# tensor4all/tensor4all-rs

Measured on AMD Instinct MI355X. Metric: TCI2 full-sweep GF/s (d=30, chi=256 fp64), higher is better.
Workload: dtype f64

## Files before the change

tensor4all-rs_amd/build.py:

```python
#!/usr/bin/env python3
import os
import subprocess
import sys
from concurrent.futures import ThreadPoolExecutor

HERE = os.path.dirname(os.path.abspath(__file__))
CSRC = os.path.join(HERE, "csrc")
OUT = os.path.join(HERE, "lib")
OBJ = os.path.join(HERE, "build")
SOURCES = ["kernels_rrlu.hip", "kernels_rrlu_reg.hip", "rrlu_xcd_plan.hip", "kernels_rrlu_xcd2.hip", "kernels_rrlu_xcd2_group.hip", "kernels_rrlu_xcd2m.hip", "kernels_rrlu_wg.hip", "kernels_rrlu_wg_group.hip", "kernels_rrlu_w1.hip", "kernels_rrlu_global.hip", "kernels_pi.hip", "kernels_chain.hip", "kernels_small.hip", "kernels_dense.hip", "kernels_linalg.hip",
           "kernels_tt.hip", "kernels_mpo.hip", "pool.hip", "engine.hip", "rook.hip", "tt.hip", "mpo.hip", "globalsearch.hip", "tci2.hip", "tci2_chain.hip", "tci2_small.hip", "conversion.hip", "patching.hip", "tree.hip", "quantics.hip", "tensorops.hip", "aci.hip", "quanticstransform.hip", "capi.hip"]
FLAGS = ["--offload-arch=gfx950", "-O3", "-std=c++17", "-fPIC", "-ffp-contract=off", "-Wall", "-Wno-unused-function",
         "-fvisibility=hidden"] + os.environ.get("T4A_EXTRA_FLAGS", "").split()
FILE_FLAGS = {"kernels_dense.hip": ["-mllvm", "-amdgpu-mfma-vgpr-form=1"], "kernels_linalg.hip": ["-ffp-contract=fast"]}
HEADERS = ["common.hpp", "stdrng.hpp", "pishard.hpp", "kernels.hpp", "kernels_rrlu_xcd_common.hpp", "kernels_rrlu_w1_body.hpp", "engine.hpp", "tci2.hpp", "tt.hpp", "mpo.hpp", "globalsearch.hpp", "rook.hpp", "patching.hpp", "tree.hpp", "quantics.hpp", "tensorops.hpp", "aci.hpp", "quanticstransform.hpp", "../../include/t4a_gpu.h",
           "../../include/t4a_testfunctions.h"]


_INC_CACHE = {}


def _includes(path):
    path = os.path.normpath(path)
    if path in _INC_CACHE:
        return _INC_CACHE[path]
    _INC_CACHE[path] = set()
    found = set()
    try:
        with open(path) as f:
            text = f.read()
    except OSError:
        return found
    import re
    for inc in re.findall(r'^\s*#\s*include\s+"([^"]+)"', text, flags=re.M):
        cand = os.path.normpath(os.path.join(os.path.dirname(path), inc))
        if os.path.exists(cand):
            found.add(cand)
            found |= _includes(cand)
    _INC_CACHE[path] = found
    return found


def _newer(target, deps):
    if not os.path.exists(target):
        return True
    t = os.path.getmtime(target)
    return any(os.path.getmtime(d) > t for d in deps)


def build(force=False, verbose=True):
    hipcc = os.environ.get("HIPCC", "/opt/rocm/bin/hipcc")
    os.makedirs(OUT, exist_ok=True)
    os.makedirs(OBJ, exist_ok=True)
    stamp = os.path.join(OBJ, "flags.stamp")
    flags_now = " ".join(FLAGS) + " | " + repr(sorted(FILE_FLAGS.items()))
    try:
        with open(stamp) as f:
            flags_then = f.read()
    except OSError:
        flags_then = None
    if flags_then != flags_now:
        force = True
    hdrs = [os.path.join(CSRC, h) for h in HEADERS]
# ... 33 lines not shown
```

tensor4all-rs_amd/csrc/kernels.hpp:

```cpp
#pragma once

#include <hip/hip_runtime.h>

#include <cstddef>
#include <cstdint>

#include "../../include/t4a_testfunctions.h"

namespace t4a {

struct RrluWorkspace;

struct RrluPlan {
    int W = 1;
    int T = 256;
    int cpw = 0;
    int Mld = 0;
    size_t lds_bytes = 0;
};

RrluPlan rrlu_make_plan(int M, int N, int num_cus);

struct RrluArgs {
    const double* A;
// ... 209 lines not shown
    const int* ldim;
    const int* woff;
    int forward, use_extras;
    int one_site;
    uint64_t* ind_code;
    uint64_t* ind_acc;
    int* ind_cnt;
    int ind_cap;
    uint64_t* dep_code;
    uint64_t* dep_acc;
    int dep_cap;
    int* rowmap;
    int* dims;
    int* hdims;
    uint64_t* snap_dst;
    int* snap_cnt_dst;
    size_t snap_words;
    int n_sites;
    uint64_t* zero_a;
    size_t zero_a_words;
    uint64_t* zero_b;
    size_t zero_b_words;
};
struct ChainPrepArgs {
    int b;
    int do_build;
    int with_rowmap;
    int prev_b;
    const int* prev_iresult;
    const int* prev_rowperm;
    const int* prev_colperm;
    unsigned prev_token;
    unsigned long long* dbg;
    int defer_host_writes;
};
struct ChainWalkArgs {
    char* blocks;
    size_t block_bytes, off_piv, off_rp, off_cp, off_ts;
    double* pi;
    int n_bonds;
    int max_steps;
    double rel_tol, abs_tol;
    double* factors;
    size_t factors_stride;
    unsigned token_base;
    int timed;
    int lean_prep;
    unsigned long long* phase_ticks;
};
void chain_walk_launch(const ChainCommon& c, const FnDevice& fn, const ChainWalkArgs& w, int columns, hipStream_t stream);
void chain_indep_launch(const ChainCommon& c, int n_bonds, hipStream_t stream);
void chain_last_core_launch(const ChainCommon& c, const FnDevice& fn, double* core, int max_entries, hipStream_t stream);
void chain_prep_launch(const ChainCommon& c, const ChainPrepArgs& a, hipStream_t stream);
void chain_pi_launch(const ChainCommon& c, const FnDevice& fn, int b, int n_dep_ub, int n_ind_ub, double* out, hipStream_t stream);

constexpr int CHAIN_GROUP_MAX = 8;
struct ChainGroupSlot {
    ChainCommon c;
    FnDevice fn;
    double* pi;
};
struct ChainPrepGroupArgs {
    ChainPrepArgs a[CHAIN_GROUP_MAX];
};
void chain_indep_group_launch(const ChainGroupSlot* d_slots, int n_handles, int n_bonds, hipStream_t stream);
void chain_prep_group_launch(const ChainGroupSlot* d_slots, const ChainPrepGroupArgs& a, int n_handles, hipStream_t stream);
void chain_pi_group_launch(const ChainGroupSlot* d_slots, int n_handles, int b, int n_dep_ub, int n_ind_ub, hipStream_t stream);

struct GemmDesc {
    int m, n, k;
    const double* A; int lda; long long strideA; int transA;
    const double* B; int ldb; long long strideB; int transB;
    double* C; int ldc; long long strideC;
    double alpha, beta;
    int batch;
    int ksplit = 1;
    double* partial = nullptr;
};
void gemm_launch(const GemmDesc& d, hipStream_t stream);

constexpr int LUCI_LEFT_CORES_MAX_JOBS = 80;
constexpr int LUCI_LEFT_CORES_MAX_RANK = 16;
struct LeftCoreJob {
    const double* lu;
    const int* dims;
    const int* iresult;
    const int* row_perm;
    double* core;
    int S;
    unsigned token;
};
struct LeftCoreJobs {
    LeftCoreJob j[LUCI_LEFT_CORES_MAX_JOBS];
};
void luci_left_cores_batched_launch(const LeftCoreJobs& jobs, int n_jobs, int max_rows, hipStream_t stream);
bool luci_factors_small_launch(const double* lu, int M, int N, int rk, const int* row_perm, const int* col_perm, bool left_orth,
                               double* left, double* right, hipStream_t stream);
void transpose_launch(const double* in, int rows, int cols, int ldi, double* out, int ldo, hipStream_t stream);

struct TrsmProblem {
    const double* T; int ldt; int n;
    double* B; int ldb; int nrhs;
    int lower; int unit_diag;
    const int* skip_flag;
};
void trsm_left_batched_launch(const TrsmProblem* d_problems, int n_problems, int max_n, int max_nrhs, hipStream_t stream);

struct LuProblem {
    double* A; int lda; int n;
    int* piv;
    int* info;
    double* B; int ldb; int nrhs;
    const unsigned long long* pmax_bits;
};
void lu_batched_launch(const LuProblem* d_problems, int n_problems, int max_n, hipStream_t stream);
constexpr int LU_MAX_PANEL_STEPS = 128;
bool lu_forward_blocked_launch(const LuProblem* d_problems, int n_problems, int max_n, int max_nrhs, hipStream_t stream, int avoid_xcc = -1,
                               unsigned* tickets = nullptr);
bool lu_solve_blocked_launch(const LuProblem* d_problems, int n_problems, int max_n, int max_nrhs, hipStream_t stream, int avoid_xcc = -1,
                             unsigned* tickets = nullptr);
// ... 118 lines not shown
```

tensor4all-rs_amd/csrc/kernels_chain.hip:

```cpp
#include "kernels.hpp"
#include "kernels_rrlu_w1_body.hpp"

namespace t4a {

namespace {

__device__ __forceinline__ const char* chain_kernarg_base()
{
#if defined(__HIP_DEVICE_COMPILE__)
    return (const char*)__builtin_amdgcn_kernarg_segment_ptr();
#else
    return nullptr;
#endif
}

constexpr int CHAIN_T = 1024;
constexpr int WALK_T = 1024;
constexpr int CHAIN_HASH = 4096;

__device__ __forceinline__ unsigned chain_hash(unsigned long long c)
{
    c ^= c >> 33;
    c *= 0xff51afd7ed558ccdull;
    c ^= c >> 29;
// ... 300 lines not shown

__device__ __forceinline__ void chain_pi_body(const ChainCommon& c, const FnDevice& fn, int b, double* __restrict__ out)
{
    const int* dm = c.dims + (size_t)b * 4;
    if (dm[2] != 0) return;
    const int K = fn.n_acc;
    const int nd = c.forward ? dm[0] : dm[1], ni = c.forward ? dm[1] : dm[0];
    const int i = blockIdx.x * blockDim.x + threadIdx.x;
    if (blockIdx.x * (int)blockDim.x >= nd) return;
    uint64_t racc[T4A_FN_MAX_ACC] = {0, 0, 0, 0};
    if (i < nd)
        for (int k = 0; k < K; ++k) racc[k] = c.dep_acc[(size_t)i * K + k];
    const uint64_t* ia = c.ind_acc + (size_t)b * c.ind_cap * K;
    for (int j = blockIdx.y; j < ni; j += gridDim.y) {
        if (i < nd) {
            uint64_t acc[T4A_FN_MAX_ACC] = {0, 0, 0, 0};
            for (int k = 0; k < K; ++k) acc[k] = racc[k] + ia[(size_t)j * K + k];
            out[(size_t)j * nd + i] = t4a_fn_value(fn.fid, acc, fn.params);
        }
    }
}
__global__ void __launch_bounds__(256) chain_pi_kernel(ChainCommon c, FnDevice fn, int b, double* __restrict__ out) { chain_pi_body(c, fn, b, out); }
__global__ void __launch_bounds__(256) chain_pi_group_kernel(const ChainGroupSlot* __restrict__ slots, int b)
{
    const ChainGroupSlot& s = slots[blockIdx.z];
    chain_pi_body(s.c, s.fn, b, s.pi);
}


__device__ __forceinline__ void chain_mirror_body(const ChainCommon& c, int nb)
{
    const int K = c.K;
    const size_t cap = (size_t)c.cap;
    const int gtid = (int)(blockIdx.x * blockDim.x + threadIdx.x), gsz = (int)(gridDim.x * blockDim.x);
    const int lane = (int)(threadIdx.x & 63), gwave = gtid >> 6, nwaves = gsz >> 6;
    for (int pf = gwave; pf < 2 * (nb + 1); pf += nwaves) {
        const int site = pf >> 1, fam = pf & 1;
        if ((fam == 0 && site == 0) || (fam == 1 && site == nb)) continue;
        const ChainTab& T = fam == 0 ? c.I : c.J;
        const ChainTab& Mr = fam == 0 ? c.mI : c.mJ;
        const int cnt = __hip_atomic_load(T.cnt + site, __ATOMIC_RELAXED, __HIP_MEMORY_SCOPE_AGENT);
        if (cnt < 0 || cnt > c.cap) continue;
        for (int e = lane; e < cnt * (1 + K); e += 64) {
            if (e < cnt) Mr.code[(size_t)site * cap + e] = T.code[(size_t)site * cap + e];
            else Mr.acc[(size_t)site * cap * K + (e - cnt)] = T.acc[(size_t)site * cap * K + (e - cnt)];
        }
        if (lane == 0) Mr.cnt[site] = cnt;
    }
    if (c.hdims)
        for (int e = gtid; e < nb * 4; e += gsz)
            if ((e & 3) != 3) c.hdims[e] = __hip_atomic_load(c.dims + e, __ATOMIC_RELAXED, __HIP_MEMORY_SCOPE_AGENT);
}

__global__ void __launch_bounds__(256) chain_last_core_kernel(ChainCommon c, FnDevice fn, double* __restrict__ core, int max_entries)
{
    const int site = c.n_sites - 1, K = c.K;
    const size_t cap = (size_t)c.cap;
    const int L = c.I.cnt[site], R = c.J.cnt[site], S = c.ldim[site], woff = c.woff[site];
    if (L < 1 || L > c.cap || R < 1 || R > c.cap || S < 1) return;
    const long long total = (long long)L * S * R;
    if (total > (long long)max_entries) return;
    for (long long e = (long long)blockIdx.x * blockDim.x + threadIdx.x; e < total; e += (long long)gridDim.x * blockDim.x) {
        const int l = (int)(e % L), s_ = (int)((e / L) % S), r = (int)(e / ((long long)L * S));
        uint64_t acc[T4A_FN_MAX_ACC] = {0, 0, 0, 0};
        for (int q = 0; q < K; ++q)
            acc[q] = c.I.acc[((size_t)site * cap + l) * K + q] + c.w[(size_t)q * c.total + woff + s_] + c.J.acc[((size_t)site * cap + r) * K + q];
        core[e] = t4a_fn_value(fn.fid, acc, fn.params);
    }
}

__device__ __forceinline__ void walk_phase_barrier(bool scalar_cache = true)
{
    if (scalar_cache) {
        __syncthreads();
        __builtin_amdgcn_s_dcache_inv();
        asm volatile("s_waitcnt lgkmcnt(0)" ::: "memory");
    } else {
        asm volatile("s_waitcnt lgkmcnt(0)\n\ts_barrier" ::: "memory");
    }
}
__device__ __forceinline__ int walk_div_small(int x, float rd) { return (int)(((float)x + 0.5f) * rd); }
__device__ __forceinline__ int walk_load_i32(const int* p) { return __hip_atomic_load(p, __ATOMIC_RELAXED, __HIP_MEMORY_SCOPE_AGENT); }

template <bool FORWARD>
__device__ __forceinline__ void walk_prep_wave0(const ChainCommon& c, WalkShared* ws, int b, int prev_b, unsigned prev_token, bool do_build, unsigned long long* dbg = nullptr)
{
    const unsigned long long dbg_t0 = dbg ? wall_clock64() : 0ull;
    const int lane = threadIdx.x & 63;
    const int K = c.K;
    const size_t cap = (size_t)c.cap;
    bool poison = false;
    int np = 0;
    if (prev_b >= 0) {
        const int pb = prev_b;
        const int pm = ws->dims[pb * 4], pn = ws->dims[pb * 4 + 1];
        const bool bad = ws->dims[pb * 4 + 2] != 0 || ws->prev_ires[1] != 0 || ws->prev_ires[3] != (int)prev_token || pm <= 0 || pn <= 0;
        const int r = ws->prev_ires[0];
        const int cnt = r > 0 ? r : 1;
        if (bad || cnt > c.cap || cnt > pm || cnt > pn || cnt > WALK_MAX_LIST) {
            poison = true;
        } else {
            const uint64_t* const pind_code = ws->ind_code[pb & 1];
            const uint64_t* const pind_acc = ws->ind_acc[pb & 1];
            uint64_t rc = 0, cc = 0, ra[T4A_FN_MAX_ACC] = {0, 0, 0, 0}, ca[T4A_FN_MAX_ACC] = {0, 0, 0, 0};
            if (lane < cnt) {
                const int ri = r > 0 ? ws->perm_rp[lane] : 0, ci = r > 0 ? ws->perm_cp[lane] : 0;
// ... 261 lines not shown
            if (tid == 0) {
                ws->prev_ires[0] = npiv >= 0 ? npiv : 0;
                ws->prev_ires[1] = npiv >= 0 ? 0 : 1;
                ws->prev_ires[2] = 0;
                ws->prev_ires[3] = npiv >= 0 ? (int)(w.token_base + (unsigned)k) : 0;
            }
        }
        walk_phase_barrier(!w.lean_prep);
        phase(2);
    }
    for (int e = tid; e < nb * 4; e += (int)blockDim.x) c.dims[e] = ws->dims[e];
    __threadfence();
    __syncthreads();
    chain_mirror_body(c, nb);
    if (w.phase_ticks && tid == 0) {
        for (int i = 0; i < 3; ++i) w.phase_ticks[i] = ph[i];
        w.phase_ticks[3] = wall_clock64() - ph_t0;
    }
}

template <int NC, bool FORWARD, bool FACTORS> void chain_walk_launch_one(const ChainCommon& c, const FnDevice& fn, const ChainWalkArgs& w, hipStream_t stream)
{
    constexpr size_t lds = walk_lds_bytes<NC, FACTORS>();
    static std::once_flag attr_once;
    std::call_once(attr_once, [] {
        (void)hipFuncSetAttribute(reinterpret_cast<const void*>(&chain_walk_kernel<NC, FORWARD, FACTORS>), hipFuncAttributeMaxDynamicSharedMemorySize, (int)lds);
    });
    hipLaunchKernelGGL((chain_walk_kernel<NC, FORWARD, FACTORS>), dim3(1), dim3(WALK_T), lds, stream, c, fn, w);
}

template <int NC> void chain_walk_launch_nc(const ChainCommon& c, const FnDevice& fn, const ChainWalkArgs& w, hipStream_t stream)
{
    if (w.factors) {
        if (c.forward) chain_walk_launch_one<NC, true, true>(c, fn, w, stream);
        else chain_walk_launch_one<NC, false, true>(c, fn, w, stream);
    } else {
        if (c.forward) chain_walk_launch_one<NC, true, false>(c, fn, w, stream);
        else chain_walk_launch_one<NC, false, false>(c, fn, w, stream);
    }
}

}

void chain_indep_launch(const ChainCommon& c, int n_bonds, hipStream_t stream)
{
    hipLaunchKernelGGL(chain_indep_kernel, dim3(n_bonds), dim3(CHAIN_T), 0, stream, c);
}

void chain_prep_launch(const ChainCommon& c, const ChainPrepArgs& a, hipStream_t stream)
{
    hipLaunchKernelGGL(chain_prep_kernel, dim3(1), dim3(CHAIN_T), 0, stream, c, a);
}

void chain_pi_launch(const ChainCommon& c, const FnDevice& fn, int b, int n_dep_ub, int n_ind_ub, double* out, hipStream_t stream)
{
    if (n_dep_ub <= 0 || n_ind_ub <= 0) return;
    const int gy = n_ind_ub < 2048 ? n_ind_ub : 2048;
    hipLaunchKernelGGL(chain_pi_kernel, dim3((n_dep_ub + 255) / 256, gy), dim3(256), 0, stream, c, fn, b, out);
}

void chain_indep_group_launch(const ChainGroupSlot* d_slots, int n_handles, int n_bonds, hipStream_t stream)
{
    hipLaunchKernelGGL(chain_indep_group_kernel, dim3(n_bonds, n_handles), dim3(CHAIN_T), 0, stream, d_slots);
}

void chain_prep_group_launch(const ChainGroupSlot* d_slots, const ChainPrepGroupArgs& a, int n_handles, hipStream_t stream)
{
    hipLaunchKernelGGL(chain_prep_group_kernel, dim3(n_handles), dim3(CHAIN_T), 0, stream, d_slots, a);
}

void chain_pi_group_launch(const ChainGroupSlot* d_slots, int n_handles, int b, int n_dep_ub, int n_ind_ub, hipStream_t stream)
{
    if (n_dep_ub <= 0 || n_ind_ub <= 0 || n_handles <= 0) return;
    const int gy = n_ind_ub < 2048 ? n_ind_ub : 2048;
    hipLaunchKernelGGL(chain_pi_group_kernel, dim3((n_dep_ub + 255) / 256, gy, n_handles), dim3(256), 0, stream, d_slots, b);
}

void chain_walk_launch(const ChainCommon& c, const FnDevice& fn, const ChainWalkArgs& w, int columns, hipStream_t stream)
{
    if (columns <= 8) chain_walk_launch_nc<8>(c, fn, w, stream);
    else if (columns <= 16) chain_walk_launch_nc<16>(c, fn, w, stream);
    else chain_walk_launch_nc<32>(c, fn, w, stream);
}

void chain_last_core_launch(const ChainCommon& c, const FnDevice& fn, double* core, int max_entries, hipStream_t stream)
{
    const int blocks = max_entries > 256 * 64 ? 64 : (max_entries + 255) / 256;
    hipLaunchKernelGGL(chain_last_core_kernel, dim3(blocks > 0 ? blocks : 1), dim3(256), 0, stream, c, fn, core, max_entries);
}

}
```

tensor4all-rs_amd/csrc/kernels_rrlu_xcd2.hip:

```cpp
#include "kernels_rrlu_xcd_common.hpp"

namespace t4a {

namespace {

template <int RPT, int KX = 1> struct Xcd2Lds {
    static constexpr int LSTR = xcd_lstr(RPT);
    static constexpr int TBL = xcd2_tbl(RPT, KX);
    static constexpr int o_l = 0;
    static constexpr int o_wd = o_l + 64 * LSTR * 8;
    static constexpr int o_wi = o_wd + 16;
    static constexpr int o_pp = o_wi + 64;
    static constexpr int o_st = o_pp + 16;
    static constexpr int o_pv = o_st + 128;
    static constexpr int o_pr = o_pv + TBL * 8;
    static constexpr int o_rp = o_pr + TBL * 2;
    static constexpr int o_pc = o_rp + TBL * 2;
    static constexpr int o_cp = o_pc + TBL * 2;
    static constexpr int bytes = o_cp + TBL * 2;
};
static_assert(Xcd2Lds<12>::bytes == (int)xcd_lds_total(12), "plan.lds_bytes must cover the layout");
static_assert(Xcd2Lds<24>::bytes == (int)xcd2_lds_total(24), "plan.lds_bytes must cover the layout (plans beyond 1024 rows)");
static_assert(Xcd2Lds<16, 3>::bytes == (int)xcd2_lds_total(16, 3), "plan.lds_bytes must cover the layout (plans beyond 1024 columns)");

#ifndef T4A_XCD_STAMP_WAVE
#define T4A_XCD_STAMP_WAVE 0
#endif

constexpr unsigned X2_META_VALID = 1u << 13;
constexpr unsigned X2_ROW_MASK = 2047u;
constexpr int X2_QSHIFT = 11, X2_PSHIFT = 11;

constexpr int X2_DIVW = XWAVES - 1;

template <int RPT, int CPT, bool ROWMAJOR, int KX = 1>
__device__ __forceinline__ void rrlu_xcd2_body(const RrluXcdArgs& p, const RrluXcdArgs* pk)
{
    static_assert(XWAVES == 8, "the second-generation kernel is written for eight waves per workgroup");
    static_assert(KX >= 1 && KX <= 3, "instantiated for up to three XCDs");
    constexpr int ST_AUX = KX > 1 ? BUF_SC1 : 0;
    extern __shared__ __attribute__((aligned(16))) char smem_raw[];
    using L = Xcd2Lds<RPT, KX>;
    constexpr int LSTR = L::LSTR;
    constexpr int MP = 64 * RPT;
    double* const lbuf = reinterpret_cast<double*>(smem_raw + L::o_l);
    int* const ctl = reinterpret_cast<int*>(smem_raw + L::o_wi);
    unsigned long long* const lds_ptrs = reinterpret_cast<unsigned long long*>(smem_raw + L::o_pp);
    unsigned long long* const lds_stamps = reinterpret_cast<unsigned long long*>(smem_raw + L::o_st);
    double* const lds_pivots = reinterpret_cast<double*>(smem_raw + L::o_pv);
    unsigned short* const posrow = reinterpret_cast<unsigned short*>(smem_raw + L::o_pr);
    unsigned short* const rowpos = reinterpret_cast<unsigned short*>(smem_raw + L::o_rp);
    unsigned short* const poscol = reinterpret_cast<unsigned short*>(smem_raw + L::o_pc);
    unsigned short* const colpos = reinterpret_cast<unsigned short*>(smem_raw + L::o_cp);

    const int tid = threadIdx.x;
    const int lane = tid & 63;
    const int wave = __builtin_amdgcn_readfirstlane(tid >> 6);
    const unsigned long long t_entry = (kXcdStamps && p.stamps) ? __builtin_amdgcn_s_memtime() : 0ull;

    if (tid == 0) {
        int rank = -1;
        if constexpr (KX == 1) {
            if ((int)xcc_id() == p.xcc) {
                const unsigned t = atomicAdd(p.ticket, 1u) - p.ticket_base;
                if (t < (unsigned)p.W) rank = (int)t;
            }
        } else {
            const unsigned x = xcc_id() & 7u;
            const unsigned t = atomicAdd(p.ticket + x, 1u) - p.ticket_base;
            const unsigned xi = (x - (unsigned)p.xcc) & 7u;
            if (xi < (unsigned)KX && t < (unsigned)p.W) rank = (int)(xi * (unsigned)p.W + t);
        }
        ctl[3] = rank;
        ctl[0] = 0;
// ... 882 lines not shown
{
    if (a.tie_row_major) xcd2_launch_tie<RPT, CPT, true>(plan, a, stream);
    else xcd2_launch_tie<RPT, CPT, false>(plan, a, stream);
}

template <int RPT> void xcd2_launch_r(const RrluXcdPlan& plan, const RrluXcdArgs& a, hipStream_t stream)
{
    switch (plan.CPT) {
    case 1: xcd2_launch_rc<RPT, 1>(plan, a, stream); break;
    case 2: xcd2_launch_rc<RPT, 2>(plan, a, stream); break;
    case 3: if constexpr (RPT * 3 <= XCD_MAX_VALUES) xcd2_launch_rc<RPT, 3>(plan, a, stream); break;
    default: if constexpr (RPT * 4 <= XCD_MAX_VALUES) xcd2_launch_rc<RPT, 4>(plan, a, stream); break;
    }
}

#else
template <int RPT, int CPT, bool ROWMAJOR>
__global__ void __launch_bounds__(XT) __attribute__((amdgpu_waves_per_eu(XWAVES / 4, XWAVES / 4))) rrlu_xcd2_group_kernel(RrluXcdGroupArgs g)
{
    (void)g;
    const unsigned x = (unsigned)__builtin_amdgcn_readfirstlane((int)xcc_id()) & 7u;
    const RrluXcdArgs* const slot = reinterpret_cast<const RrluXcdArgs*>(kernarg_base() + (size_t)x * sizeof(RrluXcdArgs));
    rrlu_xcd2_body<RPT, CPT, ROWMAJOR>(*slot, slot);
}

template <int RPT, int CPT, bool ROWMAJOR> void xcd2_group_launch_tie(const RrluXcdPlan& plan, const RrluXcdGroupArgs& a, hipStream_t stream)
{
    static std::once_flag attr_once;
    std::call_once(attr_once, [] {
        (void)hipFuncSetAttribute(reinterpret_cast<const void*>(&rrlu_xcd2_group_kernel<RPT, CPT, ROWMAJOR>),
                                  hipFuncAttributeMaxDynamicSharedMemorySize, 160 * 1024);
    });
    hipLaunchKernelGGL((rrlu_xcd2_group_kernel<RPT, CPT, ROWMAJOR>), dim3(plan.grid), dim3(XT), plan.lds_bytes, stream, a);
}
template <int RPT, int CPT> void xcd2_group_launch_rc(const RrluXcdPlan& plan, const RrluXcdGroupArgs& a, bool row_major, hipStream_t stream)
{
    if (row_major) xcd2_group_launch_tie<RPT, CPT, true>(plan, a, stream);
    else xcd2_group_launch_tie<RPT, CPT, false>(plan, a, stream);
}
template <int RPT> void xcd2_group_launch_r(const RrluXcdPlan& plan, const RrluXcdGroupArgs& a, bool row_major, hipStream_t stream)
{
    switch (plan.CPT) {
    case 1: xcd2_group_launch_rc<RPT, 1>(plan, a, row_major, stream); break;
    case 2: xcd2_group_launch_rc<RPT, 2>(plan, a, row_major, stream); break;
    case 3: if constexpr (RPT * 3 <= XCD_MAX_VALUES) xcd2_group_launch_rc<RPT, 3>(plan, a, row_major, stream); break;
    default: if constexpr (RPT * 4 <= XCD_MAX_VALUES) xcd2_group_launch_rc<RPT, 4>(plan, a, row_major, stream); break;
    }
}

#endif

}

#if defined(T4A_XCD2_MULTI_TU)
void rrlu_xcd2m_launch(const RrluXcdPlan& plan, const RrluXcdArgs& a, hipStream_t stream)
{
    const bool ok = xcd2m_launch_rc<24, 1, 1>(plan, a, stream) || xcd2m_launch_rc<24, 2, 1>(plan, a, stream) ||
                    xcd2m_launch_rc<16, 2, 3>(plan, a, stream) || xcd2m_launch_rc<24, 2, 3>(plan, a, stream) ||
                    xcd2m_launch_rc<16, 3, 2>(plan, a, stream) || xcd2m_launch_rc<24, 2, 2>(plan, a, stream);
    if (!ok) throw std::runtime_error("no kernel instantiation for this multi-XCD rrLU plan");
}
#elif !defined(T4A_XCD_GROUP_TU)
void rrlu_xcd2_launch(const RrluXcdPlan& plan, const RrluXcdArgs& a, hipStream_t stream)
{
    switch (plan.RPT) {
#ifdef T4A_XCD_DEV
    case 2: xcd2_launch_r<2>(plan, a, stream); break;
    default: xcd2_launch_r<12>(plan, a, stream); break;
#else
    case 1: xcd2_launch_r<1>(plan, a, stream); break;
    case 2: xcd2_launch_r<2>(plan, a, stream); break;
    case 3: xcd2_launch_r<3>(plan, a, stream); break;
    case 4: xcd2_launch_r<4>(plan, a, stream); break;
    case 6: xcd2_launch_r<6>(plan, a, stream); break;
    case 8: xcd2_launch_r<8>(plan, a, stream); break;
    case 12: xcd2_launch_r<12>(plan, a, stream); break;
    default: xcd2_launch_r<16>(plan, a, stream); break;
#endif
    }
}
#else
void rrlu_xcd2_group_launch(const RrluXcdPlan& plan, const RrluXcdGroupArgs& a, bool tie_row_major, hipStream_t stream)
{
    switch (plan.RPT) {
    case 1: xcd2_group_launch_r<1>(plan, a, tie_row_major, stream); break;
    case 2: xcd2_group_launch_r<2>(plan, a, tie_row_major, stream); break;
    case 3: xcd2_group_launch_r<3>(plan, a, tie_row_major, stream); break;
    case 4: xcd2_group_launch_r<4>(plan, a, tie_row_major, stream); break;
    case 6: xcd2_group_launch_r<6>(plan, a, tie_row_major, stream); break;
    case 8: xcd2_group_launch_r<8>(plan, a, tie_row_major, stream); break;
    case 12: xcd2_group_launch_r<12>(plan, a, tie_row_major, stream); break;
    default: xcd2_group_launch_r<16>(plan, a, tie_row_major, stream); break;
    }
}
#endif

}
```

tensor4all-rs_amd/csrc/rrlu_xcd_plan.hip:

```cpp
#include "kernels_rrlu_xcd_common.hpp"

namespace t4a {

namespace {

#ifdef T4A_XCD_DEV
constexpr int kRpts[] = {2, 12};
#else
constexpr int kRpts[] = {1, 2, 3, 4, 6, 8, 12, 16};
#endif
int xcd_norm_rpt(int r)
{
    for (int v : kRpts)
        if (r <= v) return v;
    return -1;
}
int xcd_norm_cpt(int c)
{
    return c <= XCD_MAX_CPT ? (c < 1 ? 1 : c) : -1;
}


}

static bool xcd_make_big_plan(int M, int N, RrluXcdPlan* out)
{
    static const bool off = std::getenv("T4A_NO_XCD_BIG") != nullptr;
    if (off || M < 1 || N < 1 || M > 1536 || N > 1536) return false;
    const int rpt = M <= 1024 ? 16 : 24;
    struct Cand { int rpt, cpt, k; };
    static const Cand cands[] = {{24, 1, 1}, {24, 2, 1}, {24, 2, 2}, {16, 2, 3}, {24, 2, 3}, {16, 3, 2}};
    static const int k_env = std::getenv("T4A_XCD_K") ? std::atoi(std::getenv("T4A_XCD_K")) : 0;
    for (const Cand& c : cands) {
        if (c.rpt != rpt) continue;
        if (k_env > 0 && c.k != k_env) continue;
        int w = (N + XWAVES * c.cpt * c.k - 1) / (XWAVES * c.cpt * c.k);
        const int wq = c.k == 3 ? 8 : c.k == 2 ? 4 : 1;
        w = (w + wq - 1) / wq * wq;
        if (w > 32) continue;
        RrluXcdPlan plan;
        plan.W = w;
        plan.RPT = c.rpt;
        plan.CPT = c.cpt;
        plan.K = c.k;
        plan.grid = 8 * w;
        plan.lds_bytes = xcd2_lds_total(c.rpt, c.k);
        *out = plan;
        return true;
    }
    return false;
}

bool rrlu_xcd_make_plan(int M, int N, RrluXcdPlan* out, bool any_size, int max_w, bool allow_big)
{
    if (max_w < 1 || max_w > 32) max_w = 32;
    if (M < 1 || N < 1) return false;
    if (M > 1024 || N > 1024) return allow_big && max_w == 32 && xcd_make_big_plan(M, N, out);
    if (!any_size && (long long)M * N <= 64 * 64) return false;
    const int rpt = xcd_norm_rpt((M + 63) / 64);
    if (rpt < 0) return false;
    int best_cpt = -1, best_w = 0;
    long best_cost = 0;
// ... 33 lines not shown
```

tensor4all-rs_amd/csrc/tci2_chain.hip:

```cpp
#include "tci2.hpp"

#include <algorithm>
#include <atomic>
#include <chrono>
#include <cmath>
#include <cstdlib>

namespace t4a {

namespace {
size_t round_up_sz(size_t v, size_t m) { return (v + m - 1) / m * m; }
std::atomic<int> g_chains_inflight{0};
}
thread_local double g_chain_wait_seconds = 0.0;

bool Tci2::chain_usable(const TCI2Options& options) const
{
    static const bool off = std::getenv("T4A_NO_CHAIN") != nullptr;
    if (off || !chain_enabled || fn_kind_ != FnKind::Builtin || options.pivot_search != 0) return false;
    long double space = 1.0L;
    for (size_t d : local_dims) space *= (long double)d;
    if (space >= 9.0e18L) return false;
    for (size_t p = 0; p < n_; ++p) {
        if (i_set[p].count == 0 || j_set[p].count == 0) return false;
// ... 439 lines not shown
        }
        if (walk) {
            ChainWalkArgs w;
            std::memset(&w, 0, sizeof(w));
            w.blocks = chain_.blocks.get();
            w.block_bytes = proto.bytes;
            w.off_piv = proto.off_piv;
            w.off_rp = proto.off_rp;
            w.off_cp = proto.off_cp;
            w.off_ts = proto.off_ts;
            w.pi = chain_.pi.get();
            w.n_bonds = (int)nb;
            w.max_steps = (int)std::min<size_t>(chi, 64);
            w.rel_tol = chain_.tol;
            w.abs_tol = chain_.one_site ? chain_.abs_tol : 0.0;
            w.factors = chain_.factors_stride ? chain_.factors.get() : nullptr;
            w.factors_stride = chain_.factors_stride;
            if (chain_.walk_token > 0xFFFF0000u || chain_.walk_token == 0u) chain_.walk_token = 1u;
            w.token_base = chain_.walk_token;
            chain_.walk_token += (unsigned)nb;
            w.timed = chain_.timed ? 1 : 0;
            w.lean_prep = 1;
            static const bool walk_dbg = std::getenv("T4A_WALK_DEBUG") != nullptr;
            if (walk_dbg) {
                chain_.walk_dbg.reserve(8);
                T4A_HIP(hipMemsetAsync(chain_.walk_dbg.get(), 0, 8 * sizeof(unsigned long long), st));
                w.phase_ticks = chain_.walk_dbg.get();
            }
            chain_.walked = true;
            for (size_t k = 0; k < nb; ++k) tokens[order[k]] = w.token_base + (unsigned)k;
            chain_walk_launch(c, fn_dev_, w, (int)walk_cols, st);
            ++chain_stats_ext[0];
        }
        static const bool want_prep_dbg = std::getenv("T4A_PREP_DEBUG") != nullptr;
        unsigned long long* prep_dbg = nullptr;
        if (want_prep_dbg && !walk) {
            chain_.walk_dbg.reserve(8);
            T4A_HIP(hipMemsetAsync(chain_.walk_dbg.get(), 0, 8 * sizeof(unsigned long long), st));
            prep_dbg = chain_.walk_dbg.get();
            chain_.prep_dbg = true;
        }
        bool spec_pending = false;
        for (size_t k = 0; !walk && k < nb; ++k) {
            const size_t b = order[k];
            const RrluRoute& pl = plans[b];
            const bool fused = pl.fused;
            const bool spec_here = spec_pending && !fused;
            const RrluBlock blk = block_of(b);
            ChainPrepArgs pa;
            std::memset(&pa, 0, sizeof(pa));
            pa.b = (int)b;
            pa.do_build = 1;
            pa.dbg = prep_dbg;
            pa.defer_host_writes = 0;
            pa.with_rowmap = spec_here ? 1 : 0;
            pa.prev_b = -1;
            if (k > 0) {
                const size_t pb = order[k - 1];
                const RrluBlock pblk = block_of(pb);
                pa.prev_b = (int)pb;
                pa.prev_iresult = pblk.iresult();
                pa.prev_rowperm = pblk.row_perm();
                pa.prev_colperm = pblk.col_perm();
                pa.prev_token = tokens[pb];
            }
            chain_prep_launch(c, pa, st);
            if (!fused && !spec_here) chain_pi_launch(c, fn_dev_, (int)b, (int)dep_ub[b], (int)ind_ub[b], chain_.pi.get(), st);
            XcdSpecArgs sp;
            std::memset(&sp, 0, sizeof(sp));
            spec_pending = false;
            if (solo && k + 1 < nb && pl.on_xcd()) {
                const size_t nx = order[k + 1];
                if (!plans[nx].fused) {
                    const size_t site = forward ? nx : nx + 1;
                    const ChainTab& H = forward ? c.HI : c.HJ;
                    const size_t hsite = forward ? nx + 1 : nx;
                    sp.out = chain_.spec[(k + 1) & 1].get();
                    sp.dep_acc = c.dep_acc;
                    sp.w_site = c.w + offset_[site];
                    sp.ext_acc = H.acc + hsite * cap * K;
                    sp.ext_cnt = use_extras ? H.cnt + hsite : nullptr;
                    sp.ind_acc = c.ind_acc + nx * ind_cap * K;
                    sp.ind_cnt = c.ind_cnt + nx;
                    sp.tile_counter = tile_counters + nx;
                    sp.total = (int)total_;
                    sp.d = (int)local_dims[site];
                    sp.fn = fn_dev_;
                    spec_pending = true;
                }
            }
            FusedPi fp;
            fp.fn = fn_dev_;
            fp.d_rowacc = c.dep_acc;
            fp.d_colacc = c.ind_acc + b * ind_cap * K;
            fp.host_resident = false;
            const double* A = fused ? nullptr : (spec_here ? chain_.spec[k & 1].get() : chain_.pi.get());
            if (timed_events) T4A_HIP(hipEventRecord(chain_.t0[b], st));
            tokens[b] = eng.chain_rrlu(pl, forward, A, spec_here ? c.rowmap : nullptr, fused ? &fp : nullptr, c.dims + b * 4, chi, chain_.tol,
                                       chain_.one_site ? chain_.abs_tol : 0.0, blk, spec_pending ? &sp : nullptr,
                                       chain_.factors_stride ? chain_.factors.get() + b * chain_.factors_stride : nullptr, chain_.urows.get());
            if (timed_events) T4A_HIP(hipEventRecord(chain_.t1[b], st));
        }
        if (!walk) {
            const size_t pb = order[nb - 1];
            const RrluBlock pblk = block_of(pb);
            ChainPrepArgs pa;
            std::memset(&pa, 0, sizeof(pa));
            pa.do_build = 0;
            pa.defer_host_writes = 0;
            pa.prev_b = (int)pb;
            pa.prev_iresult = pblk.iresult();
            pa.prev_rowperm = pblk.row_perm();
            pa.prev_colperm = pblk.col_perm();
            pa.prev_token = tokens[pb];
            chain_prep_launch(c, pa, st);
        }
        chain_.cores_batched = false;
        if (chain_.one_site && chain_.factors_stride && forward && nb <= (size_t)LUCI_LEFT_CORES_MAX_JOBS) {
            LeftCoreJobs jobs;
            std::memset(&jobs, 0, sizeof(jobs));
            size_t max_rows = 1;
            for (size_t b = 0; b < nb; ++b) {
                const RrluBlock blk = block_of(b);
                const size_t rub = std::max<size_t>(std::min({dep_ub[b], ind_ub[b], chi}), 1);
                DevCore& core = cores[b];
                core.buf.reserve(std::max<size_t>(dep_ub[b] * rub, 1));
                LeftCoreJob& j = jobs.j[b];
                j.lu = chain_.factors.get() + b * chain_.factors_stride;
                j.dims = c.dims + b * 4;
                j.iresult = blk.iresult();
                j.row_perm = blk.row_perm();
                j.core = core.buf.get();
                j.S = (int)local_dims[b];
                j.token = tokens[b];
                max_rows = std::max(max_rows, dep_ub[b]);
            }
            luci_left_cores_batched_launch(jobs, (int)nb, (int)max_rows, st);
            chain_.cores_batched = true;
        }
        chain_.last_core_launched = false;
        if (chain_.one_site && chain_.factors_stride && forward) {
            const size_t last = n_ - 1;
            const size_t a_ub = std::max<size_t>(std::min({dep_ub[nb - 1], ind_ub[nb - 1], chi}), 1);
            const size_t entries = a_ub * local_dims[last] * std::max<size_t>(j_set[last].count, 1);
            if (entries <= ((size_t)1 << 24)) {
                cores[last].buf.reserve(entries);
                chain_last_core_launch(c, fn_dev_, cores[last].buf.get(), (int)entries, st);
                chain_.last_core_launched = true;
            }
        }
        T4A_HIP(hipMemcpyAsync(chain_.hblocks.get(), chain_.blocks.get(), nb * proto.bytes, hipMemcpyDeviceToHost, st));
        T4A_HIP(hipGetLastError());
    } catch (...) {
        (void)hipStreamSynchronize(st);
        eng.chain_end();
        if (counted) g_chains_inflight.fetch_sub(1);
        chain_.tables_valid = false;
        chain_.snap_serial[0] = chain_.snap_serial[1] = ~0ull;
        throw;
    }
    chain_.inflight = true;
    chain_.wait_stream = st;
    chain_.group_role = 0;
}

void Tci2::chain_group_launch(const std::vector<Tci2*>& hs)
{
    const size_t nh = hs.size();
// ... 29 lines not shown
    size_t reserve_words = 0;
    {
        const RrluRoute cr = side_ub ? Engine::chain_group_route((int)side_ub, (int)side_ub) : RrluRoute();
        if (cr.ok()) reserve_words = cr.xcd_mailbox_words();
    }
    std::vector<char> counted(nh, 0);
    bool locked = false;
    try {
        lead->chain_.gslots.reserve(CHAIN_GROUP_MAX);
        lead->chain_.hgslots.reserve(CHAIN_GROUP_MAX);
        for (size_t i = 0; i < nh; ++i) {
            Tci2* h = hs[i];
            h->chain_.prepared = false;
            if (h != lead) {
                if (!h->chain_.group_ev) T4A_HIP(hipEventCreateWithFlags(&h->chain_.group_ev, hipEventDisableTiming));
                T4A_HIP(hipEventRecord(h->chain_.group_ev, h->eng.stream()));
                T4A_HIP(hipStreamWaitEvent(st, h->chain_.group_ev, 0));
            }
            h->eng.chain_group_reserve(gplans, reserve_words, st);
            ChainGroupSlot& slot = lead->chain_.hgslots.get()[i];
            slot.c = h->chain_.common;
            slot.fn = h->fn_dev_;
            slot.pi = h->chain_.pi.get();
            g_chains_inflight.fetch_add(1);
            counted[i] = 1;
        }
        T4A_HIP(hipMemcpyAsync(lead->chain_.gslots.get(), lead->chain_.hgslots.get(), nh * sizeof(ChainGroupSlot), hipMemcpyHostToDevice, st));
        const ChainGroupSlot* d_slots = lead->chain_.gslots.get();
        lead->eng.chain_group_lock();
        locked = true;
        auto block_of = [&](Tci2* h, size_t b) {
            RrluBlock k = h->chain_.proto;
            k.dev = h->chain_.blocks.get() + b * k.bytes;
            return k;
        };
        auto prev_of = [&](Tci2* h, size_t pb, ChainPrepArgs& pa) {
            const RrluBlock pblk = block_of(h, pb);
            pa.prev_b = (int)pb;
            pa.prev_iresult = pblk.iresult();
            pa.prev_rowperm = pblk.row_perm();
            pa.prev_colperm = pblk.col_perm();
            pa.prev_token = h->chain_.tokens[pb];
        };
        chain_indep_group_launch(d_slots, (int)nh, (int)nb, st);
        const std::vector<size_t>& order = lead->chain_.order;
        for (size_t k = 0; k < nb; ++k) {
            const size_t b = order[k];
            ChainPrepGroupArgs pg;
            std::memset(&pg, 0, sizeof(pg));
            for (size_t i = 0; i < nh; ++i) {
                ChainPrepArgs& pa = pg.a[i];
                pa.b = (int)b;
                pa.do_build = 1;
                pa.prev_b = -1;
                if (k > 0) prev_of(hs[i], order[k - 1], pa);
            }
            chain_prep_group_launch(d_slots, pg, (int)nh, st);
            chain_pi_group_launch(d_slots, (int)nh, (int)b, gplans[b].kM, gplans[b].kN, st);
            RrluXcdGroupArgs ga;
            std::memset(&ga, 0, sizeof(ga));
            for (int x = 0; x < 8; ++x) ga.p[x].xcc = -1;
            for (size_t i = 0; i < nh; ++i) {
                Tci2* h = hs[i];
                h->chain_.tokens[b] = h->eng.chain_group_args(gplans[b], forward, h->chain_.pi.get(), h->chain_.common.dims + b * 4, h->chain_.chi,
                                                              h->chain_.tol, 0.0, block_of(h, b), (int)i, &ga.p[i], st);
            }
            gplans[b].launch_group(ga, !forward, st);
        }
        {
            ChainPrepGroupArgs pg;
            std::memset(&pg, 0, sizeof(pg));
            for (size_t i = 0; i < nh; ++i) prev_of(hs[i], order[nb - 1], pg.a[i]);
            chain_prep_group_launch(d_slots, pg, (int)nh, st);
        }
        for (Tci2* h : hs)
            T4A_HIP(hipMemcpyAsync(h->chain_.hblocks.get(), h->chain_.blocks.get(), nb * h->chain_.proto.bytes, hipMemcpyDeviceToHost, st));
        T4A_HIP(hipGetLastError());
    } catch (...) {
        (void)hipStreamSynchronize(st);
        if (locked) lead->eng.chain_end();
        for (size_t i = 0; i < nh; ++i) {
            if (counted[i]) g_chains_inflight.fetch_sub(1);
            hs[i]->chain_.prepared = false;
            hs[i]->chain_.tables_valid = false;
            hs[i]->chain_.snap_serial[0] = hs[i]->chain_.snap_serial[1] = ~0ull;
        }
        throw;
    }
    for (Tci2* h : hs) {
        h->chain_.plans = gplans;
        h->chain_.inflight = true;
        h->chain_.wait_stream = st;
        h->chain_.group_role = h == lead ? 1 : 2;
    }
}

void Tci2::chain_abort() noexcept
{
    if (chain_.prepared) {
        chain_.snap_serial[0] = chain_.snap_serial[1] = ~0ull;
        chain_.tables_valid = false;
    }
    chain_.prepared = false;
    chain_.walked = false;
    if (!chain_.inflight) return;
    chain_.inflight = false;
    hipStream_t st = chain_.wait_stream ? chain_.wait_stream : eng.stream();
    (void)hipStreamSynchronize(st);
    (void)hipGetLastError();
    if (chain_.group_role != 2) eng.chain_end();
    chain_.group_role = 0;
    chain_.wait_stream = nullptr;
    g_chains_inflight.fetch_sub(1);
    chain_.tables_valid = false;
    chain_.snap_serial[0] = chain_.snap_serial[1] = ~0ull;
}

void Tci2::chain_finish(const TCI2Options& options)
{
    if (!chain_.inflight) return;
    chain_.inflight = false;
    hipStream_t st = chain_.wait_stream ? chain_.wait_stream : eng.stream();
    const size_t nb = n_ - 1;
    const size_t K = (size_t)chain_.n_acc, cap = chain_.cap;
    const bool forward = chain_.forward;
    const RrluBlock& proto = chain_.proto;
// ... 238 lines not shown
```

Baseline: 303.4.

## Defer host-mirror writes to one final mirror kernel and add fitted rrLU row-slot instantiations

Chain prep kernels now defer their writes to the host-visible dims mirror. A single mirror kernel (single-handle and grouped versions) copies the dims once after the last prep, instead of every per-bond prep writing to host memory. Separately, rrLU row-per-thread choices 5, 7, 9, 10 and 11 are added to the plan set and instantiated in new translation units, so plans can fit the row count more tightly. This adds more kernel instantiations and build time, and the planner may now pick new kernel shapes with different occupancy.

```diff
diff --git a/tensor4all-rs_amd/build.py b/tensor4all-rs_amd/build.py
--- a/tensor4all-rs_amd/build.py
+++ b/tensor4all-rs_amd/build.py
@@ -8,7 +8,7 @@
 CSRC = os.path.join(HERE, "csrc")
 OUT = os.path.join(HERE, "lib")
 OBJ = os.path.join(HERE, "build")
-SOURCES = ["kernels_rrlu.hip", "kernels_rrlu_reg.hip", "rrlu_xcd_plan.hip", "kernels_rrlu_xcd2.hip", "kernels_rrlu_xcd2_group.hip", "kernels_rrlu_xcd2m.hip", "kernels_rrlu_wg.hip", "kernels_rrlu_wg_group.hip", "kernels_rrlu_w1.hip", "kernels_rrlu_global.hip", "kernels_pi.hip", "kernels_chain.hip", "kernels_small.hip", "kernels_dense.hip", "kernels_linalg.hip",
+SOURCES = ["kernels_rrlu.hip", "kernels_rrlu_reg.hip", "rrlu_xcd_plan.hip", "kernels_rrlu_xcd2.hip", "kernels_rrlu_xcd2_fit.hip", "kernels_rrlu_xcd2_group.hip", "kernels_rrlu_xcd2_group_fit.hip", "kernels_rrlu_xcd2m.hip", "kernels_rrlu_wg.hip", "kernels_rrlu_wg_group.hip", "kernels_rrlu_w1.hip", "kernels_rrlu_global.hip", "kernels_pi.hip", "kernels_chain.hip", "kernels_small.hip", "kernels_dense.hip", "kernels_linalg.hip",
            "kernels_tt.hip", "kernels_mpo.hip", "pool.hip", "engine.hip", "rook.hip", "tt.hip", "mpo.hip", "globalsearch.hip", "tci2.hip", "tci2_chain.hip", "tci2_small.hip", "conversion.hip", "patching.hip", "tree.hip", "quantics.hip", "tensorops.hip", "aci.hip", "quanticstransform.hip", "capi.hip"]
 FLAGS = ["--offload-arch=gfx950", "-O3", "-std=c++17", "-fPIC", "-ffp-contract=off", "-Wall", "-Wno-unused-function",
          "-fvisibility=hidden"] + os.environ.get("T4A_EXTRA_FLAGS", "").split()
diff --git a/tensor4all-rs_amd/csrc/kernels.hpp b/tensor4all-rs_amd/csrc/kernels.hpp
--- a/tensor4all-rs_amd/csrc/kernels.hpp
+++ b/tensor4all-rs_amd/csrc/kernels.hpp
@@ -285,6 +285,7 @@
 void chain_indep_launch(const ChainCommon& c, int n_bonds, hipStream_t stream);
 void chain_last_core_launch(const ChainCommon& c, const FnDevice& fn, double* core, int max_entries, hipStream_t stream);
 void chain_prep_launch(const ChainCommon& c, const ChainPrepArgs& a, hipStream_t stream);
+void chain_mirror_launch(const ChainCommon& c, int n_bonds, hipStream_t stream);
 void chain_pi_launch(const ChainCommon& c, const FnDevice& fn, int b, int n_dep_ub, int n_ind_ub, double* out, hipStream_t stream);
 
 constexpr int CHAIN_GROUP_MAX = 8;
@@ -299,6 +300,7 @@
 void chain_indep_group_launch(const ChainGroupSlot* d_slots, int n_handles, int n_bonds, hipStream_t stream);
 void chain_prep_group_launch(const ChainGroupSlot* d_slots, const ChainPrepGroupArgs& a, int n_handles, hipStream_t stream);
 void chain_pi_group_launch(const ChainGroupSlot* d_slots, int n_handles, int b, int n_dep_ub, int n_ind_ub, hipStream_t stream);
+void chain_mirror_group_launch(const ChainGroupSlot* d_slots, int n_handles, int n_bonds, hipStream_t stream);
 
 struct GemmDesc {
     int m, n, k;
diff --git a/tensor4all-rs_amd/csrc/kernels_chain.hip b/tensor4all-rs_amd/csrc/kernels_chain.hip
--- a/tensor4all-rs_amd/csrc/kernels_chain.hip
+++ b/tensor4all-rs_amd/csrc/kernels_chain.hip
@@ -376,6 +376,12 @@
             if ((e & 3) != 3) c.hdims[e] = __hip_atomic_load(c.dims + e, __ATOMIC_RELAXED, __HIP_MEMORY_SCOPE_AGENT);
 }
 
+__global__ void __launch_bounds__(256) chain_mirror_kernel(ChainCommon c, int nb) { chain_mirror_body(c, nb); }
+__global__ void __launch_bounds__(256) chain_mirror_group_kernel(const ChainGroupSlot* __restrict__ slots, int nb)
+{
+    chain_mirror_body(slots[blockIdx.y].c, nb);
+}
+
 __global__ void __launch_bounds__(256) chain_last_core_kernel(ChainCommon c, FnDevice fn, double* __restrict__ core, int max_entries)
 {
     const int site = c.n_sites - 1, K = c.K;
@@ -743,6 +749,11 @@
     hipLaunchKernelGGL(chain_prep_kernel, dim3(1), dim3(CHAIN_T), 0, stream, c, a);
 }
 
+void chain_mirror_launch(const ChainCommon& c, int n_bonds, hipStream_t stream)
+{
+    hipLaunchKernelGGL(chain_mirror_kernel, dim3((2 * (n_bonds + 1) + 3) / 4), dim3(256), 0, stream, c, n_bonds);
+}
+
 void chain_pi_launch(const ChainCommon& c, const FnDevice& fn, int b, int n_dep_ub, int n_ind_ub, double* out, hipStream_t stream)
 {
     if (n_dep_ub <= 0 || n_ind_ub <= 0) return;
@@ -760,6 +771,12 @@
     hipLaunchKernelGGL(chain_prep_group_kernel, dim3(n_handles), dim3(CHAIN_T), 0, stream, d_slots, a);
 }
 
+void chain_mirror_group_launch(const ChainGroupSlot* d_slots, int n_handles, int n_bonds, hipStream_t stream)
+{
+    if (n_handles <= 0) return;
+    hipLaunchKernelGGL(chain_mirror_group_kernel, dim3((2 * (n_bonds + 1) + 3) / 4, n_handles), dim3(256), 0, stream, d_slots, n_bonds);
+}
+
 void chain_pi_group_launch(const ChainGroupSlot* d_slots, int n_handles, int b, int n_dep_ub, int n_ind_ub, hipStream_t stream)
 {
     if (n_dep_ub <= 0 || n_ind_ub <= 0 || n_handles <= 0) return;
diff --git a/tensor4all-rs_amd/csrc/kernels_rrlu_xcd2.hip b/tensor4all-rs_amd/csrc/kernels_rrlu_xcd2.hip
--- a/tensor4all-rs_amd/csrc/kernels_rrlu_xcd2.hip
+++ b/tensor4all-rs_amd/csrc/kernels_rrlu_xcd2.hip
@@ -20,6 +20,9 @@
     static constexpr int bytes = o_cp + TBL * 2;
 };
 static_assert(Xcd2Lds<12>::bytes == (int)xcd_lds_total(12), "plan.lds_bytes must cover the layout");
+static_assert(Xcd2Lds<5>::bytes == (int)xcd_lds_total(5) && Xcd2Lds<7>::bytes == (int)xcd_lds_total(7) && Xcd2Lds<9>::bytes == (int)xcd_lds_total(9) &&
+                  Xcd2Lds<10>::bytes == (int)xcd_lds_total(10) && Xcd2Lds<11>::bytes == (int)xcd_lds_total(11),
+              "plan.lds_bytes must cover the layout (fitted row-slot counts)");
 static_assert(Xcd2Lds<24>::bytes == (int)xcd2_lds_total(24), "plan.lds_bytes must cover the layout (plans beyond 1024 rows)");
 static_assert(Xcd2Lds<16, 3>::bytes == (int)xcd2_lds_total(16, 3), "plan.lds_bytes must cover the layout (plans beyond 1024 columns)");
 
@@ -1008,6 +1011,9 @@
 
 }
 
+void rrlu_xcd2_fit_launch(const RrluXcdPlan& plan, const RrluXcdArgs& a, hipStream_t stream);
+void rrlu_xcd2_group_fit_launch(const RrluXcdPlan& plan, const RrluXcdGroupArgs& a, bool tie_row_major, hipStream_t stream);
+
 #if defined(T4A_XCD2_MULTI_TU)
 void rrlu_xcd2m_launch(const RrluXcdPlan& plan, const RrluXcdArgs& a, hipStream_t stream)
 {
@@ -1017,6 +1023,19 @@
     if (!ok) throw std::runtime_error("no kernel instantiation for this multi-XCD rrLU plan");
 }
 #elif !defined(T4A_XCD_GROUP_TU)
+#if defined(T4A_XCD_FIT_TU)
+void rrlu_xcd2_fit_launch(const RrluXcdPlan& plan, const RrluXcdArgs& a, hipStream_t stream)
+{
+    switch (plan.RPT) {
+    case 5: xcd2_launch_r<5>(plan, a, stream); break;
+    case 7: xcd2_launch_r<7>(plan, a, stream); break;
+    case 9: xcd2_launch_r<9>(plan, a, stream); break;
+    case 10: xcd2_launch_r<10>(plan, a, stream); break;
+    case 11: xcd2_launch_r<11>(plan, a, stream); break;
+    default: throw std::runtime_error("no kernel instantiation for this fitted single-XCD rrLU plan");
+    }
+}
+#else
 void rrlu_xcd2_launch(const RrluXcdPlan& plan, const RrluXcdArgs& a, hipStream_t stream)
 {
     switch (plan.RPT) {
@@ -1031,8 +1050,23 @@
     case 6: xcd2_launch_r<6>(plan, a, stream); break;
     case 8: xcd2_launch_r<8>(plan, a, stream); break;
     case 12: xcd2_launch_r<12>(plan, a, stream); break;
-    default: xcd2_launch_r<16>(plan, a, stream); break;
+    case 16: xcd2_launch_r<16>(plan, a, stream); break;
+    default: rrlu_xcd2_fit_launch(plan, a, stream); break;
 #endif
+    }
+}
+#endif
+#else
+#if defined(T4A_XCD_FIT_TU)
+void rrlu_xcd2_group_fit_launch(const RrluXcdPlan& plan, const RrluXcdGroupArgs& a, bool tie_row_major, hipStream_t stream)
+{
+    switch (plan.RPT) {
+    case 5: xcd2_group_launch_r<5>(plan, a, tie_row_major, stream); break;
+    case 7: xcd2_group_launch_r<7>(plan, a, tie_row_major, stream); break;
+    case 9: xcd2_group_launch_r<9>(plan, a, tie_row_major, stream); break;
+    case 10: xcd2_group_launch_r<10>(plan, a, tie_row_major, stream); break;
+    case 11: xcd2_group_launch_r<11>(plan, a, tie_row_major, stream); break;
+    default: throw std::runtime_error("no kernel instantiation for this fitted single-XCD rrLU group plan");
     }
 }
 #else
@@ -1046,9 +1080,11 @@
     case 6: xcd2_group_launch_r<6>(plan, a, tie_row_major, stream); break;
     case 8: xcd2_group_launch_r<8>(plan, a, tie_row_major, stream); break;
     case 12: xcd2_group_launch_r<12>(plan, a, tie_row_major, stream); break;
-    default: xcd2_group_launch_r<16>(plan, a, tie_row_major, stream); break;
+    case 16: xcd2_group_launch_r<16>(plan, a, tie_row_major, stream); break;
+    default: rrlu_xcd2_group_fit_launch(plan, a, tie_row_major, stream); break;
     }
 }
 #endif
-
-}
+#endif
+
+}
diff --git a/tensor4all-rs_amd/csrc/kernels_rrlu_xcd2_fit.hip b/tensor4all-rs_amd/csrc/kernels_rrlu_xcd2_fit.hip
--- /dev/null
+++ b/tensor4all-rs_amd/csrc/kernels_rrlu_xcd2_fit.hip
@@ -0,0 +1,2 @@
+#define T4A_XCD_FIT_TU 1
+#include "kernels_rrlu_xcd2.hip"
diff --git a/tensor4all-rs_amd/csrc/kernels_rrlu_xcd2_group_fit.hip b/tensor4all-rs_amd/csrc/kernels_rrlu_xcd2_group_fit.hip
--- /dev/null
+++ b/tensor4all-rs_amd/csrc/kernels_rrlu_xcd2_group_fit.hip
@@ -0,0 +1,3 @@
+#define T4A_XCD_GROUP_TU 1
+#define T4A_XCD_FIT_TU 1
+#include "kernels_rrlu_xcd2.hip"
diff --git a/tensor4all-rs_amd/csrc/rrlu_xcd_plan.hip b/tensor4all-rs_amd/csrc/rrlu_xcd_plan.hip
--- a/tensor4all-rs_amd/csrc/rrlu_xcd_plan.hip
+++ b/tensor4all-rs_amd/csrc/rrlu_xcd_plan.hip
@@ -7,7 +7,7 @@
 #ifdef T4A_XCD_DEV
 constexpr int kRpts[] = {2, 12};
 #else
-constexpr int kRpts[] = {1, 2, 3, 4, 6, 8, 12, 16};
+constexpr int kRpts[] = {1, 2, 3, 4, 5, 6, 7, 8, 9, 10, 11, 12, 16};
 #endif
 int xcd_norm_rpt(int r)
 {
diff --git a/tensor4all-rs_amd/csrc/tci2_chain.hip b/tensor4all-rs_amd/csrc/tci2_chain.hip
--- a/tensor4all-rs_amd/csrc/tci2_chain.hip
+++ b/tensor4all-rs_amd/csrc/tci2_chain.hip
@@ -515,7 +515,7 @@
             pa.b = (int)b;
             pa.do_build = 1;
             pa.dbg = prep_dbg;
-            pa.defer_host_writes = 0;
+            pa.defer_host_writes = 1;
             pa.with_rowmap = spec_here ? 1 : 0;
             pa.prev_b = -1;
             if (k > 0) {
@@ -570,13 +570,14 @@
             ChainPrepArgs pa;
             std::memset(&pa, 0, sizeof(pa));
             pa.do_build = 0;
-            pa.defer_host_writes = 0;
+            pa.defer_host_writes = 1;
             pa.prev_b = (int)pb;
             pa.prev_iresult = pblk.iresult();
             pa.prev_rowperm = pblk.row_perm();
             pa.prev_colperm = pblk.col_perm();
             pa.prev_token = tokens[pb];
             chain_prep_launch(c, pa, st);
+            chain_mirror_launch(c, (int)nb, st);
         }
         chain_.cores_batched = false;
         if (chain_.one_site && chain_.factors_stride && forward && nb <= (size_t)LUCI_LEFT_CORES_MAX_JOBS) {
@@ -712,6 +713,7 @@
                 ChainPrepArgs& pa = pg.a[i];
                 pa.b = (int)b;
                 pa.do_build = 1;
+                pa.defer_host_writes = 1;
                 pa.prev_b = -1;
                 if (k > 0) prev_of(hs[i], order[k - 1], pa);
             }
@@ -730,8 +732,12 @@
         {
             ChainPrepGroupArgs pg;
             std::memset(&pg, 0, sizeof(pg));
-            for (size_t i = 0; i < nh; ++i) prev_of(hs[i], order[nb - 1], pg.a[i]);
+            for (size_t i = 0; i < nh; ++i) {
+                pg.a[i].defer_host_writes = 1;
+                prev_of(hs[i], order[nb - 1], pg.a[i]);
+            }
             chain_prep_group_launch(d_slots, pg, (int)nh, st);
+            chain_mirror_group_launch(d_slots, (int)nh, (int)nb, st);
         }
         for (Tci2* h : hs)
             T4A_HIP(hipMemcpyAsync(h->chain_.hblocks.get(), h->chain_.blocks.get(), nb * h->chain_.proto.bytes, hipMemcpyDeviceToHost, st));
```

New measurement: 304.8 (median of 6 runs). Within noise of the previous version (+0.5%).
